# eanswer/TactileSimulation

Hardware: AMD Instinct MI355X
Metric: env-steps/sec (fwd+bwd) TactilePush batch=4096 (higher is better)
Workload: dtype f32

## Files before the change

include/tsim.h:

```cpp
#ifndef TSIM_H
#define TSIM_H
#include <stdint.h>
#ifdef __cplusplus
extern "C" {
#endif

typedef struct tsim_batch tsim_batch;
enum { TSIM_F32 = 0, TSIM_F64 = 1 };

int tsim_batch_create(const int32_t* I, const double* F, int B, int tape_capacity, int dtype, int device,
                      tsim_batch** out);
void tsim_batch_destroy(tsim_batch* b);

int tsim_ndof_r(const tsim_batch* b);
int tsim_ndof_u(const tsim_batch* b);
int tsim_ndof_var(const tsim_batch* b);
int tsim_ndof_tactile(const tsim_batch* b);
int tsim_batch_size(const tsim_batch* b);
int tsim_dtype(const tsim_batch* b);
double tsim_timestep(const tsim_batch* b);
int tsim_tape_len(const tsim_batch* b);

int tsim_update_model(tsim_batch* b, const int32_t* I, const double* F, void* stream);

// ... 57 lines not shown
                    void* g_out, void* H_out, long long* cycles, void* stream);

int tsim_debug_signature(tsim_batch* b, int t_first, int n, uint32_t* out, void* stream);

int tsim_debug_stamps(tsim_batch* b, long long* cycles);

int tsim_launch_info(const tsim_batch* b, int32_t* out);
enum { TSIM_KT_FORWARD = 0, TSIM_KT_TAXELS = 1, TSIM_KT_BACKWARD = 2, TSIM_KT_COUNT = 3 };
int tsim_kernel_timing(tsim_batch* b, int enable);
int tsim_kernel_times(tsim_batch* b, double* ms_sum, int32_t* launches);
int tsim_set_lanes_per_env(tsim_batch* b, int lanes);
int tsim_static_model(const tsim_batch* b);
int tsim_set_static(tsim_batch* b, int allow);
const char* tsim_kernel_variant(const tsim_batch* b);
enum { TSIM_OPT_PAIR_CULL = 1, TSIM_OPT_VALUE_TRIALS = 2, TSIM_OPT_TRIAL_HELPERS = 3, TSIM_OPT_VALUE_FIRST = 4, TSIM_OPT_CROSS_KINKS = 5, TSIM_OPT_EVAL_BUDGET = 6,
       TSIM_OPT_ALL_DEFAULT = 7, TSIM_OPT_FRAME_RECORDS = 8 };
int tsim_set_option(tsim_batch* b, int option, int value);
int tsim_get_option(const tsim_batch* b, int option);

int tsim_last_evals(tsim_batch* b, int32_t* host_out);
int tsim_last_helper_trials(tsim_batch* b, int32_t* host_out);

#define TSIM_KINK_FACTOR 1000.0
#define TSIM_KINK_LS 4
#define TSIM_KINK_MAX 6
int tsim_set_solver_options(tsim_batch* b, int cross_kinks, int eval_budget);
int tsim_last_gnorm(tsim_batch* b, float* host_out);

const char* tsim_last_error(void);

#ifdef __cplusplus
// ... 4 lines not shown
```

tactilesimulation_amd/csrc/tsim_batch.h:

```cpp
#pragma once
#include <hip/hip_runtime.h>
#include <cstdint>
#include <string>
#include <vector>
#include "../../include/tsim.h"
#include "tsim_launch.h"

static thread_local std::string g_err;
static int fail(const std::string& m) { g_err = m; return 1; }
#define HIPCHK(x) do { hipError_t e_ = (x); if (e_ != hipSuccess) return fail(std::string(#x) + ": " + hipGetErrorString(e_)); } while (0)

struct DeviceGuard {
  int prev = -1; bool ok = true;
  explicit DeviceGuard(int dev) {
    if (hipGetDevice(&prev) != hipSuccess) prev = -1;
    if (prev != dev) ok = hipSetDevice(dev) == hipSuccess; else prev = -1;
  }
  ~DeviceGuard() { if (prev >= 0) (void)hipSetDevice(prev); }
};
#define TS_DEVICE(b) DeviceGuard guard_((b)->device); if (!guard_.ok) return fail("hipSetDevice(" + std::to_string((b)->device) + ") failed")

static bool capturing(hipStream_t st) {
  hipStreamCaptureStatus cs = hipStreamCaptureStatusNone;
  return hipStreamIsCapturing(st, &cs) != hipSuccess || cs != hipStreamCaptureStatusNone;
// ... 28 lines not shown
  DevBuf evals;
  DevBuf helped;
  DevBuf gnorm;
  int cross_kinks = 0, eval_budget = 0;
  DevBuf order; int order_valid = 0;
  DevBuf order_ep; int order_ep_n = 0;
  DevBuf prev; int has_prev = 0;
  DevBuf poseR, poseD; int nspt;
  int has_exp;
  int t_cur, record;
  int lpe_forced;
  int nsched;
  int stage_cpt;
  int n_simd;
  int last_frame_rec = 0;
  int value_trials = 2;
  int trial_helpers = 1;
  int value_first = 1;
  bool ab_no_episode_lpt = false, ab_inkernel_readout = false, ab_no_free_run = false, ab_lockstep = false, ab_taxels_per_record = false, ab_no_envtab_cpt = false, ab_no_default_opts = false, ab_inkernel_frame_out = false; int ab_bwd_lpe = 0, ab_lpt_deal = 2;
  int pair_cull = 1;
  int static_id = 0, static_exact = 0, env_struct_ok = 0, no_static = 0;
  DevBuf dKmask, dFlag;
  DevBuf fposeR, fposeD; int fpose_frames = 0;
  int pose_valid = 0;
  int pose_off = 0;
  int tt_off = 0;
  int tax_slots = 0;
  size_t esz;
  std::vector<CacheEntry> cache;
  std::vector<void*> pool;
  std::vector<void*> retired;
  long long* bwd_stamps = nullptr;
  void* dLdp = nullptr; DevBuf zbuf, pgpart; int pg_chunks = 0;
  int pg_groups = TS_PG_CONTACT; DevBuf pgbpart;
  DevBuf tan_src; size_t tan_src_reals = 0; int tan_src_captured = 0;
  DevBuf pg_slots;
  int adj_kernel = -1, adj_passes = 0;
  int kt_on = 0;
  std::vector<KtPair> kt;
  std::vector<hipEvent_t> kt_free;
};
template <class F> static auto by_real(const tsim_batch* b, F&& f) { return by_dtype(b->dtype, f); }

struct KtScope {
  tsim_batch* b; hipStream_t st; KtPair p; bool on = false;
  KtScope(tsim_batch* b_, int kind, hipStream_t st_) : b(b_), st(st_) {
    if (!b->kt_on || b->kt.size() >= (size_t)1 << 16) return;
    if (capturing(st)) return;
    hipEvent_t e[2];
    for (int i = 0; i < 2; ++i) {
      if (!b->kt_free.empty()) { e[i] = b->kt_free.back(); b->kt_free.pop_back(); }
      else if (hipEventCreate(&e[i]) != hipSuccess) { (void)hipGetLastError(); if (i) b->kt_free.push_back(e[0]); return; }
    }
    p.a = e[0]; p.b = e[1]; p.kind = kind;
    on = hipEventRecord(p.a, st) == hipSuccess;
    if (!on) { b->kt_free.push_back(e[0]); b->kt_free.push_back(e[1]); }
  }
// ... 24 lines not shown
```

tactilesimulation_amd/csrc/tsim_hip.hip:

```cpp
#include <hip/hip_runtime.h>
#include <cstdio>
#include <cstdlib>
#include <cstring>
#include <cmath>
#include <algorithm>
#include <string>
#include <vector>
#include "../../include/tsim.h"
#include "tsim_eval.h"
#include "tsim_policy_push.h"
#include "tsim_static_pusher.h"


#include "tsim_kernels.h"
#include "tsim_param_grad.h"
#include "tsim_launch.h"
#include "tsim_batch.h"

__global__ void __launch_bounds__(1024) k_order_by_evals(const int* evals, int* order, int B, int ns, int lo, int span, int deal) {
  __shared__ int hist[64], base[64];
  const int t = threadIdx.x;
  if (t < 64) hist[t] = 0;
  __syncthreads();
  auto bin = [lo, span](int ev) { return min(max((ev - lo) * 64 / span, 0), 63); };
// ... 159 lines not shown
  for (int t = (int)blockIdx.y * a.slice + (int)threadIdx.x; t < te; t += 256 * TS_TAX_UNROLL) {
    V3<R> xa[TS_TAX_UNROLL];
#pragma unroll
    for (int r = 0; r < TS_TAX_UNROLL; ++r) {
      const int tr = min(t + 256 * r, te - 1);
      xa[r] = mk3<R>(tax[tr], tax[tr + ntax], tax[tr + 2 * ntax]);
    }
#pragma unroll
    for (int r = 0; r < TS_TAX_UNROLL; ++r)
      if (t + 256 * r < te) taxel(t + 256 * r, xa[r]);
  }
}

enum { TXS_RPB = 16, TXS_MAXK = 8, TXS_MAXS = 4, TXS_MAX_TAXELS = 1024 };
template <class R>
__global__ void __launch_bounds__(256) k_taxels_small(TaxArgs<R> a, int nrec) {
  const int rec0 = blockIdx.x * TXS_RPB, nr_ = min((int)TXS_RPB, nrec - rec0);
  const int ntax = a.ntax, nsensor = a.nsensor, nspt = a.nspt;
  __shared__ int sEnd[TXS_MAXS], sKb[TXS_MAXS], sNsp[TXS_MAXS], sPrim[TXS_MAXK], sPair[TXS_MAXK], sSlot[TXS_RPB];
  __shared__ R sSf[TXS_RPB][TXS_MAXS * TSIM_SF_SIZE], sShape[TXS_RPB][TXS_MAXK * 4], sP[TXS_RPB][TXS_MAXK * TP_R_SIZE];
  __shared__ double sD[TXS_RPB][TXS_MAXK * TP_D_SIZE];
  __shared__ __attribute__((aligned(16))) R sC[TXS_RPB][TXS_MAXK * 4];
  __shared__ R sX[3 * TXS_MAX_TAXELS];
  const R* tax = a.F + a.foff_taxel;
  for (int i = threadIdx.x; i < 3 * ntax; i += 256) sX[i] = tax[i];
  const int* TT = a.I + a.tt_off;
  for (int i = threadIdx.x; i < nsensor; i += 256) { sEnd[i] = TT[3 * i]; sKb[i] = TT[3 * i + 1]; sNsp[i] = TT[3 * i + 2]; }
  for (int i = threadIdx.x; i < nspt; i += 256) { sPrim[i] = TT[3 * nsensor + 2 * i]; sPair[i] = TT[3 * nsensor + 2 * i + 1]; }
  for (int i = threadIdx.x; i < nr_; i += 256) { const int fr = (rec0 + i) / a.B; sSlot[i] = a.tac_slot ? a.tac_slot[fr] : fr; }
  for (int i = threadIdx.x; i < nr_ * nspt * TP_R_SIZE; i += 256) { const int r = i / (nspt * TP_R_SIZE), e = i % (nspt * TP_R_SIZE); sP[r][e] = a.poseR[(size_t)(rec0 + r) * nspt * TP_R_SIZE + e]; }
  for (int i = threadIdx.x; i < nr_ * nspt * TP_D_SIZE; i += 256) { const int r = i / (nspt * TP_D_SIZE), e = i % (nspt * TP_D_SIZE); sD[r][e] = a.poseD[(size_t)(rec0 + r) * nspt * TP_D_SIZE + e]; }
  for (int i = threadIdx.x; i < nr_ * nsensor * TSIM_SF_SIZE; i += 256) {
    const int r = i / (nsensor * TSIM_SF_SIZE), e = i % (nsensor * TSIM_SF_SIZE);
    const R* F = a.Fenv ? a.Fenv + (size_t)((rec0 + r) % a.B) * a.fstride : a.F;
    sSf[r][e] = F[a.foff_sensor + e];
  }
  __syncthreads();
  for (int i = threadIdx.x; i < nr_ * nspt * 4; i += 256) {
    const int r = i / (nspt * 4), e = i % (nspt * 4);
    const R* F = a.Fenv ? a.Fenv + (size_t)((rec0 + r) % a.B) * a.fstride : a.F;
    sShape[r][e] = F[a.foff_pair + sPair[e >> 2] * TSIM_PF_SIZE + TSIM_PF_SHAPE + (e & 3)];
  }
  __syncthreads();
  for (int i = threadIdx.x; i < nr_ * nspt; i += 256) { const int r = i / nspt, k = i % nspt; taxel_bound<R>(sP[r] + k * TP_R_SIZE, sPrim[k], sShape[r] + k * 4, sC[r] + 4 * k); }
  __syncthreads();
  for (int item = threadIdx.x; item < nr_ * ntax; item += 256) {
    const int r = item / ntax, t = item - r * ntax;
    const int tslot = sSlot[r];
    if (tslot < 0) continue;
    R* out = a.tac_out + ((size_t)tslot * a.B + (rec0 + r) % a.B) * 3 * ntax;
    taxel_eval<R>(t, mk3<R>(sX[t], sX[t + ntax], sX[t + 2 * ntax]), nsensor, sEnd, sKb, sNsp, sPrim, sSf[r], sShape[r], sP[r], sD[r], sC[r], tax, ntax, out);
  }
}

template <class R> struct SigArgs { const int* I; const R* F; const R* Fenv; int fstride; int B, t_first, n; const R* tape; unsigned* out; int stage_cpt; int tk; };

__device__ __forceinline__ unsigned wave_sum_u32(unsigned x) {
  for (int off = 32; off > 0; off >>= 1) x += (unsigned)lane_gather((int)x, (int)threadIdx.x ^ off);
  return x;
}

template <class R>
__global__ void __launch_bounds__(TS_WAVE) k_signature(SigArgs<R> a) {
  extern __shared__ __attribute__((aligned(16))) unsigned char smem_raw[];
  R* lds = reinterpret_cast<R*>(smem_raw);
// ... 337 lines not shown
}
template <class R> static BwdArgs<R> bwd_args(const tsim_batch* b) {
  BwdArgs<R> a{};
  a.I = b->dI; a.F = (const R*)b->dF; a.Fenv = (const R*)b->dFenv; a.fstride = b->nfrec; a.B = b->B; a.t_end = b->t_cur;
  a.tape = (const R*)b->tape; a.lamq = (R*)b->lamq; a.lamv = (R*)b->lamv; a.stage_cpt = b->stage_cpt; a.cull = b->pair_cull; a.tk = b->tape_k;
  return a;
}

enum { TS_POSE_EMIT_MIN_TAXELS = 4096 };
static bool pose_emit(tsim_batch* b, hipStream_t st) {
  pose_invalidate(b, st);
  return !b->pose_off && b->nspt > 0 && b->poseR && b->ntax >= TS_POSE_EMIT_MIN_TAXELS;
}

static bool taxels_supported(const tsim_batch* b) { return b->ntax > 0 && b->nspt > 0 && b->nspt <= TX_MAXK && b->I[TSIM_IH_NSENSOR] <= TX_MAXS; }
template <class R>
static int launch_taxels(tsim_batch* b, const void* poseR, const double* poseD, int frames, const int32_t* tac_slot, void* tac_out, hipStream_t st) {
  if (b->tax_slots == 0) {
    int per_cu = 0;
    const hipError_t e_ = hipOccupancyMaxActiveBlocksPerMultiprocessor(&per_cu, k_taxels<R>, 256, 0);
    b->tax_slots = (e_ == hipSuccess && per_cu > 0 ? per_cu : 4) * (b->n_simd / 4);
  }
  const long long nrec = (long long)frames * b->B;
  if (nrec >= 4 * TXS_RPB && b->ntax <= TXS_MAX_TAXELS && b->nspt <= TXS_MAXK && b->I[TSIM_IH_NSENSOR] <= TXS_MAXS && !b->ab_taxels_per_record) {
    TaxArgs<R> t{b->dI, (const R*)b->dF, (const R*)b->dFenv, b->nfrec, (const R*)poseR, poseD, b->nspt, (R*)tac_out, 0, b->B, tac_slot,
                 b->ntax, b->I[TSIM_IH_NSENSOR], b->I[TSIM_IH_FOFF_SENSOR], b->I[TSIM_IH_FOFF_PAIR], b->I[TSIM_IH_FOFF_TAXEL], b->tt_off};
    hipLaunchKernelGGL(k_taxels_small<R>, dim3((unsigned)((nrec + TXS_RPB - 1) / TXS_RPB)), dim3(256), 0, st, t, (int)nrec);
    HIPCHK(hipGetLastError());
    return 0;
  }
  const int per_env = (int)std::max<long long>(1, std::min<long long>(b->tax_slots / nrec, (b->ntax + 255) / 256));
  const int slice = ((b->ntax + per_env - 1) / per_env + 255) / 256 * 256;
  const dim3 tgrid((unsigned)nrec, (b->ntax + slice - 1) / slice);
  TaxArgs<R> t{b->dI, (const R*)b->dF, (const R*)b->dFenv, b->nfrec, (const R*)poseR, poseD, b->nspt, (R*)tac_out, slice, b->B, tac_slot,
               b->ntax, b->I[TSIM_IH_NSENSOR], b->I[TSIM_IH_FOFF_SENSOR], b->I[TSIM_IH_FOFF_PAIR], b->I[TSIM_IH_FOFF_TAXEL], b->tt_off};
  hipLaunchKernelGGL(k_taxels<R>, tgrid, dim3(256), 0, st, t);
  HIPCHK(hipGetLastError());
  return 0;
}

template <class R>
static int launch_forward(tsim_batch* b, const void* u, int nframes, const int32_t* tac_slot, int nsub, void* q_out, void* qd_out, void* var_out, void* tac_out, int32_t* status, hipStream_t st) {
  FwdArgs<R> a = fwd_args<R>(b);
  a.nsub = nsub; a.nframes = nframes; a.tac_slot = tac_slot; a.u = (const R*)u;
  a.q_out = (R*)q_out; a.qd_out = (R*)qd_out; a.var_out = (R*)var_out; a.tac_out = (R*)tac_out; a.status = status;
// ... 14 lines not shown
      if (rc) defer = false;
    }
  }
  if (defer) { a.fposeR = (R*)b->fposeR; a.fposeD = b->fposeD; }
  a.free_run = (defer || !tac_out || b->ntax == 0) && !b->ab_no_free_run;
  a.lockstep = b->ab_lockstep ? 1 : 0;
  if (a.lockstep) a.free_run = 0;
  TsPlan plan = ts_plan(b, TS_K_FORWARD, false, 0);
  if (b->record && !plan.fused) b->tape_k_ok = 0;
  const TsPlan fr_plan = ts_plan(b, TS_K_FRAME_RECORDS, false, 0);
  const bool frame_rec = defer && a.free_run && b->record && nframes > 1 && plan.fused && !emit && !b->ab_inkernel_frame_out &&
                         fr_plan.variant == plan.variant && fr_plan.lpe == plan.lpe;
  a.frame_rec = frame_rec ? 1 : 0;
  plan.frame_rec = frame_rec;
  b->last_frame_rec = !frame_rec ? 0 : (plan.frame_rec && plan.default_opts) ? 2 : 1;
  { KtScope kt_(b, TSIM_KT_FORWARD, st); if (!ts_launch<false, R>(plan, st, a)) return fail("no k_forward instantiation for the launch plan"); }
  HIPCHK(hipGetLastError());
  if (defer) {
    KtScope kt_(b, TSIM_KT_TAXELS, st);
    if (frame_rec) {
      TsPlan p = fr_plan;
      const int nblk = (int)p.grid, chunks = std::max(1, std::min(nframes, b->n_simd / std::max(nblk, 1))), fpc = (nframes + chunks - 1) / chunks;
      p.grid = (unsigned)(nblk * ((nframes + fpc - 1) / fpc));
      if (!ts_launch<false, R>(p, st, a, fpc)) return fail("no k_frame_records instantiation for the launch plan");
      HIPCHK(hipGetLastError());
    }
    if (launch_taxels<R>(b, b->fposeR, b->fposeD, nframes, tac_slot, tac_out, st)) return 1;
  }
  b->pose_valid = emit ? 1 : 0;
  if (b->B >= 256) {
    const int ns = TS_WAVE / plan.lpe, nsv = (b->B % ns == 0) ? ns : 1;
    if (nframes > 1) {
      const int n = nframes * nsub;
      hipLaunchKernelGGL(k_order_by_evals, dim3(1), dim3(1024), 0, st, (const int*)b->evals, b->order_ep, b->B, nsv, 2 * n, std::max(1, 5 * n / 2), b->ab_lpt_deal);
      b->order_ep_n = n; b->order_valid = 0;
    } else {
      hipLaunchKernelGGL(k_order_by_evals, dim3(1), dim3(1024), 0, st, (const int*)b->evals, b->order, b->B, nsv, 0, 64, b->ab_lpt_deal);
      b->order_valid = 1;
    }
    HIPCHK(hipGetLastError());
  } else if (nframes > 1) b->order_valid = 0;
  return 0;
// ... 246 lines not shown
  b->rec = ts_rec(nr, nu, (int)b->esz, b->tape_k);
  if (lds_bytes_for(b, 1) > 64 * 1024) { delete b; return fail("model needs more than 64 KiB of LDS per environment"); }
  decide_stage_cpt(b);
  b->nspt = b->I[TSIM_IH_NSPRIM];
  size_t tape_bytes = (size_t)(tape_capacity + 1) * B * b->rec * b->esz;
  if (hipMalloc(&b->dI, (b->I.size() + b->nsched) * sizeof(int32_t)) != hipSuccess || hipMalloc(&b->dF, b->F.size() * b->esz) != hipSuccess ||
      hipMalloc(&b->tape, tape_bytes) != hipSuccess || hipMalloc(&b->lamq, (size_t)2 * B * nr * b->esz) != hipSuccess ||
      hipMalloc(&b->lamv, (size_t)2 * B * nr * b->esz) != hipSuccess || hipMalloc(&b->evals, (size_t)B * sizeof(int)) != hipSuccess || hipMalloc((void**)&b->helped, (size_t)B * sizeof(int)) != hipSuccess || hipMemset(b->helped, 0, (size_t)B * sizeof(int)) != hipSuccess || hipMalloc((void**)&b->gnorm, (size_t)B * sizeof(float)) != hipSuccess || hipMalloc(&b->order, (size_t)B * sizeof(int)) != hipSuccess || hipMalloc((void**)&b->order_ep, (size_t)B * sizeof(int)) != hipSuccess || hipMalloc(&b->prev, (size_t)B * 2 * nr * sizeof(double)) != hipSuccess ||
      (b->nspt > 0 && (hipMalloc(&b->poseR, (size_t)B * b->nspt * TP_R_SIZE * b->esz) != hipSuccess || hipMalloc((void**)&b->poseD, (size_t)B * b->nspt * TP_D_SIZE * sizeof(double)) != hipSuccess))) {
    tsim_batch_destroy(b);
    return fail("hipMalloc failed (tape bytes = " + std::to_string(tape_bytes) + ")");
  }
  if (hipMemset(b->tape, 0, tape_bytes) != hipSuccess || hipMemset(b->lamq, 0, (size_t)2 * B * nr * b->esz) != hipSuccess ||
      hipMemset(b->lamv, 0, (size_t)2 * B * nr * b->esz) != hipSuccess) { tsim_batch_destroy(b); return fail("hipMemset failed"); }
  if (upload_model(b, nullptr)) { tsim_batch_destroy(b); return 1; }
  *out = b;
  return 0;
}

void tsim_batch_destroy(tsim_batch* b) {
  if (!b) return;
  DeviceGuard guard_(b->device);
  for (auto& e : b->cache) (void)hipFree(e.buf);
  for (void* p : b->pool) (void)hipFree(p);
  for (void* p : b->retired) (void)hipFree(p);
  for (auto& k : b->kt) { (void)hipEventDestroy(k.a); (void)hipEventDestroy(k.b); }
  for (hipEvent_t e : b->kt_free) (void)hipEventDestroy(e);
  (void)hipFree(b->tape);
  delete b;
}

int tsim_ndof_r(const tsim_batch* b) { return b->nr; }
int tsim_ndof_u(const tsim_batch* b) { return b->nu; }
int tsim_ndof_var(const tsim_batch* b) { return 3 * b->nvar; }
int tsim_ndof_tactile(const tsim_batch* b) { return 3 * b->ntax; }
int tsim_batch_size(const tsim_batch* b) { return b->B; }
int tsim_dtype(const tsim_batch* b) { return b->dtype; }
double tsim_timestep(const tsim_batch* b) { return b->F[TSIM_FH_H]; }
int tsim_tape_len(const tsim_batch* b) { return b->record ? b->t_cur : 0; }
int tsim_launch_info(const tsim_batch* b, int32_t* out) { return plan_info(ts_plan(b, TS_K_FORWARD, false, 0), out); }
int tsim_tangent_launch_info(const tsim_batch* b, int ndir, int with_dtables, int32_t* out) {
  if (!b || !out) return fail("tangent_launch_info: null argument");
// ... 49 lines not shown
  if (option == TSIM_OPT_PAIR_CULL) { b->pair_cull = value != 0; return 0; }
  if (option == TSIM_OPT_VALUE_TRIALS) { if (value < 0) return fail("set_option: TSIM_OPT_VALUE_TRIALS >= 0"); b->value_trials = value; return 0; }
  if (option == TSIM_OPT_TRIAL_HELPERS) { b->trial_helpers = value != 0; return 0; }
  if (option == TSIM_OPT_VALUE_FIRST) { b->value_first = value != 0; return 0; }
  return fail("set_option: unknown option " + std::to_string(option));
}
int tsim_get_option(const tsim_batch* b, int option) {
  if (option == TSIM_OPT_PAIR_CULL) return b->pair_cull;
  if (option == TSIM_OPT_VALUE_TRIALS) return b->value_trials;
  if (option == TSIM_OPT_TRIAL_HELPERS) return b->trial_helpers;
  if (option == TSIM_OPT_VALUE_FIRST) return b->value_first;
  if (option == TSIM_OPT_CROSS_KINKS) return b->cross_kinks;
  if (option == TSIM_OPT_EVAL_BUDGET) return b->eval_budget;
  if (option == TSIM_OPT_ALL_DEFAULT) return default_options(b) ? 1 : 0;
  if (option == TSIM_OPT_FRAME_RECORDS) return b->last_frame_rec;
  return -1;
}
int tsim_set_solver_options(tsim_batch* b, int cross_kinks, int eval_budget) {
  if (eval_budget < 0) return fail("set_solver_options: negative evaluation budget");
  b->cross_kinks = cross_kinks != 0;
  b->eval_budget = eval_budget;
  return 0;
}
int tsim_last_gnorm(tsim_batch* b, float* host_out) {
  TS_DEVICE(b);
  if (hipMemcpy(host_out, b->gnorm, (size_t)b->B * sizeof(float), hipMemcpyDeviceToHost) != hipSuccess) return fail("last_gnorm: copy failed");
  return 0;
}
int tsim_last_helper_trials(tsim_batch* b, int32_t* host_out) {
  TS_DEVICE(b);
// ... 364 lines not shown
```

tactilesimulation_amd/csrc/tsim_kernels.h:

```cpp
#pragma once
#include <hip/hip_runtime.h>
#include "../../include/tsim.h"
#include "tsim_eval.h"
#include "tsim_policy_push.h"

template <class MS, class C> __device__ __forceinline__ int ts_integrator(const C& c) {
  if constexpr (std::is_void<MS>::value) return ts_u(c.I[TSIM_IH_INTEGRATOR]); else return MS::Iv(TSIM_IH_INTEGRATOR);
}
template <class MS> constexpr int ts_static_nr() { if constexpr (std::is_void<MS>::value) return 0; else return MS::Iv(TSIM_IH_NR); }

__host__ __device__ inline int ts_qw(int esz) { return 8 / esz; }
__host__ __device__ inline int ts_rec(int nr, int nu, int esz, int tk) { return (ts_qw(esz) * nr + nr + nr * nr + nu + (tk ? nr * nr : 0) + 1) & ~1; }
template <class R> __device__ __forceinline__ double* rec_q(R* rec) { return reinterpret_cast<double*>(rec); }
template <class R> __device__ __forceinline__ const double* rec_q(const R* rec) { return reinterpret_cast<const double*>(rec); }
template <class R> __device__ __forceinline__ int rec_qd(int nr) { return ts_qw((int)sizeof(R)) * nr; }
template <class R> __device__ __forceinline__ int rec_H(int nr) { return ts_qw((int)sizeof(R)) * nr + nr; }
template <class R> __device__ __forceinline__ int rec_u(int nr) { return ts_qw((int)sizeof(R)) * nr + nr + nr * nr; }
template <class R> __device__ __forceinline__ int rec_K(int nr, int nu) { return ts_qw((int)sizeof(R)) * nr + nr + nr * nr + nu; }

template <int LPE, class R>
__device__ __forceinline__ void readout(const Ctx<R>& c, int lane, int env, bool wr_var, bool wr, bool has_var, bool has_tac, R* var_out, R* tac_out, int tb = 0, int te = 0x7fffffff) {
  if (has_var && wr_var) {
    for (int e = lane; e < c.nvar; e += LPE) {
      const int l = c.I[c.off_var + e * TSIM_VI_SIZE + TSIM_VI_LINK];
// ... 35 lines not shown
        R o0 = R(0), o1 = R(0), o2 = R(0);
        if (Fl.x != R(0) || Fl.y != R(0) || Fl.z != R(0)) {
          o0 = Fl.x * tp[3 * c.ntax] + Fl.y * tp[4 * c.ntax] + Fl.z * tp[5 * c.ntax];
          o1 = Fl.x * tp[6 * c.ntax] + Fl.y * tp[7 * c.ntax] + Fl.z * tp[8 * c.ntax];
          o2 = Fl.x * tp[9 * c.ntax] + Fl.y * tp[10 * c.ntax] + Fl.z * tp[11 * c.ntax];
        }
        if (j0 == 0) { o[0] = o0; o[1] = o1; o[2] = o2; } else { o[0] += o0; o[1] += o1; o[2] += o2; }
      }
    }
  }
}

__device__ __forceinline__ float ts_trial_point(float base, float alpha, float dq) { return __builtin_fmaf(alpha, dq, base); }
__device__ __forceinline__ double ts_trial_point(double base, double alpha, double dq) { return __builtin_fma(alpha, dq, base); }
enum { TP_R_SIZE = 18, TP_D_SIZE = 12 };
template <class R> struct FwdArgs {
  const int* I; const R* F; const R* Fenv; int fstride;
  int B, nsub, record, t0;
  int tk = 0;
  int nframes;
  const int* tac_slot;
  R* tape; const R* u;
  R *q_out, *qd_out, *var_out, *tac_out; int* status; int* evals;
  const int* order;
  double* prev; int has_prev;
  int stage_cpt;
  int cross_kinks;
  int eval_budget;
  float* gnorm;
  PushPolicy<R> pol;
// ... 362 lines not shown
#ifdef TS_ROUND_STATS
    if (lane == 0) { if (a.gnorm) a.gnorm[env] = (float)(clock64() - rs_t0_); if (a.status) a.status[env] = rounds_; }
    if (lane == 0 && a.helped) a.helped[env] = (int)(fe_cycles_ < (1ll << 23) - 1 ? fe_cycles_ : (1ll << 23) - 1) * 256 + (fe_execs_ < 255 ? fe_execs_ : 255);
#endif
  }
}
#undef helpers_on
#undef TS_OPT
#undef TS_RECORD
template <class R, int NRM, bool EXPJ, int LPE, bool POLICY = false, class MS = void>
__global__ void TS_KLB k_forward(FwdArgs<R> a) { ts_forward<R, NRM, EXPJ, LPE, POLICY, MS>(a); }
template <class R, int NRM, int LPE, class MS>
__global__ void TS_KLB k_forward_fr(FwdArgs<R> a) { ts_forward<R, NRM, false, LPE, false, TsFrameRecords<TsDefaultOpts<MS>>>(a); }

template <class R, int LPE, class MS>
__global__ void TS_KLB k_frame_records(FwdArgs<R> a, int fpc) {
  extern __shared__ __attribute__((aligned(16))) unsigned char smem_raw[];
  R* lds = reinterpret_cast<R*>(smem_raw);
  constexpr int NS = TS_WAVE / LPE;
  const int slot = threadIdx.x / LPE, lane = threadIdx.x % LPE;
  const int nblk = (a.B + NS - 1) / NS, chunk = blockIdx.x / nblk;
  const int eidx = (blockIdx.x - chunk * nblk) * NS + slot;
  const bool valid = eidx < a.B;
  const int env = min(eidx, a.B - 1);
  Ctx<R> c; ctx_init<R, MS>(c, a.I, a.F, lds, NS, slot, lane, LPE, false, a.Fenv ? a.Fenv + (size_t)env * a.fstride : nullptr);
  const int nr = c.nr, REC = ts_rec(nr, c.nu, (int)sizeof(R), a.tk);
  init_world(c, lane, LPE);
  const int f0 = chunk * fpc, f1 = min(f0 + fpc, a.nframes);
  double qn = 0.0; R qdn = R(0);
  const R* st = a.tape + ((size_t)(a.t0 + (f0 + 1) * a.nsub) * a.B + env) * REC;
  const size_t frame_stride = (size_t)a.nsub * a.B * REC;
  if (f0 < f1 && lane < nr) { qn = rec_q(st)[lane]; qdn = st[rec_qd<R>(nr) + lane]; }
  for (int f = f0; f < f1; ++f) {
    const int tslot = a.tac_slot ? a.tac_slot[f] : f;
    TS_SYNC();
    if (lane < nr) { c.qD[lane] = qn; c.q0D[lane] = qn; c.q[lane] = (R)qn; c.qd[lane] = qdn; c.qd0[lane] = qdn; c.qa[lane] = R(0); }
    st += frame_stride;
    if (f + 1 < f1 && lane < nr) { qn = rec_q(st)[lane]; qdn = st[rec_qd<R>(nr) + lane]; }
    TS_SYNC();
// ... 279 lines not shown
```

tactilesimulation_amd/csrc/tsim_launch.h:

```cpp
#pragma once
#include <type_traits>
#include "tsim_kernels.h"
#include "tsim_param_grad.h"
#include "tsim_tangent.h"
#include "tsim_tangent_closed.h"
#include "tsim_frame_jacobian.h"
#include "tsim_tactile_jacobian.h"
#include "tsim_param_jacobian.h"
#include "tsim_static_pusher.h"

enum TsKernel { TS_K_FORWARD, TS_K_BACKWARD, TS_K_BACKWARD_Z, TS_K_DEBUG_EVAL, TS_K_PARAM_GRAD, TS_K_PARAM_GRAD_BODY, TS_K_FRAME_RECORDS,
                TS_K_CLOSED_BACKWARD_Z,
                TS_K_TANGENT,
                TS_K_TANGENT_BODY,
                TS_K_CLOSED_TANGENT,
                TS_K_FRAME_JACOBIAN,
                TS_K_TACTILE_JACOBIAN,
                TS_K_PARAM_JACOBIAN };
enum { TS_KM_GENERIC = 0, TS_KM_STATIC = 1, TS_KM_PARAM = 2 };
using TsParamPusher = TsParam<TsStaticPusher>;

struct TsPlan {
  int kernel = TS_K_FORWARD, variant = TS_KM_GENERIC;
  int nrm = 8; bool expj = false; int lpe = TS_WAVE;
// ... 32 lines not shown
template <int N> using TsInt = std::integral_constant<int, N>;
template <bool B> using TsBool = std::integral_constant<bool, B>;

template <class MS, bool POLICY, class R> struct TsLaunch {
  template <int K, class F> static bool shape(const TsPlan& p, F&& f) {
    if (p.kernel != K || p.policy != POLICY) return false;
    auto at = [&](auto nrm, auto expj, auto lpe) {
      if constexpr (ts_instantiated(K, ts_view_nrm<MS>(), sizeof(R) == 4, POLICY, false, nrm, expj, lpe)) { f(nrm, expj, lpe); return true; }
      else return false;
    };
    auto lanes = [&](auto nrm, auto expj) { return p.lpe == 16 ? at(nrm, expj, TsInt<16>()) : p.lpe == 32 ? at(nrm, expj, TsInt<32>()) : p.lpe == 64 && at(nrm, expj, TsInt<64>()); };
    if (p.expj) return p.nrm == 16 && lanes(TsInt<16>(), TsBool<true>());
    return p.nrm == 8 ? lanes(TsInt<8>(), TsBool<false>()) : p.nrm == 16 && lanes(TsInt<16>(), TsBool<false>());
  }
  static bool run(const TsPlan& p, hipStream_t st, const FwdArgs<R>& a);
  static bool run(const TsPlan& p, hipStream_t st, const FwdArgs<R>& a, int fpc);
  static bool run(const TsPlan& p, hipStream_t st, const BwdArgs<R>& a, R* zsave = nullptr);
  static bool run_closed_z(const TsPlan& p, hipStream_t st, const BwdArgs<R>& a, R* zsave);
  static bool run(const TsPlan& p, hipStream_t st, const DbgArgs<R>& a);
  static bool run(const TsPlan& p, hipStream_t st, const PgArgs<R>& a);
  static bool run(const TsPlan& p, hipStream_t st, const PgBodyArgs<R>& a);
  static bool run(const TsPlan& p, hipStream_t st, const TanArgs<R>& a);
  static bool run(const TsPlan& p, hipStream_t st, const TanBodyArgs<R>& a);
  static bool run(const TsPlan& p, hipStream_t st, const FjArgs<R>& a);
  static bool run(const TsPlan& p, hipStream_t st, const TjArgs<R>& a);
  static bool run(const TsPlan& p, hipStream_t st, const PjArgs<R>& a);
  static bool run_tangent_src(const TsPlan& p, hipStream_t st, const TanArgs<R>& a);
  static bool run_closed_tangent(const TsPlan& p, hipStream_t st, const TanClosedArgs<R>& a);
};

template <class MS, bool POLICY, class R> bool TsLaunch<MS, POLICY, R>::run(const TsPlan& p, hipStream_t st, const FwdArgs<R>& a) {
  return shape<TS_K_FORWARD>(p, [&](auto nrm, auto expj, auto lpe) {
    if constexpr (ts_instantiated(TS_K_FORWARD, ts_view_nrm<MS>(), sizeof(R) == 4, POLICY, true, nrm, expj, lpe)) {
      if (p.default_opts && p.frame_rec) {
        if constexpr (!POLICY && ts_static_fused<MS, R>()) { hipLaunchKernelGGL((k_forward_fr<R, nrm, lpe, MS>), dim3(p.grid), dim3(TS_WAVE), p.lds, st, a); return; }
      }
      if (p.default_opts) { hipLaunchKernelGGL((k_forward<R, nrm, expj, lpe, POLICY, TsDefaultOpts<MS>>), dim3(p.grid), dim3(TS_WAVE), p.lds, st, a); return; }
    }
    hipLaunchKernelGGL((k_forward<R, nrm, expj, lpe, POLICY, MS>), dim3(p.grid), dim3(TS_WAVE), p.lds, st, a);
  });
}
template <class MS, bool POLICY, class R> bool TsLaunch<MS, POLICY, R>::run(const TsPlan& p, hipStream_t st, const FwdArgs<R>& a, int fpc) {
  if constexpr (!POLICY && ts_static_fused<MS, R>())
    return shape<TS_K_FRAME_RECORDS>(p, [&](auto, auto, auto lpe) { hipLaunchKernelGGL((k_frame_records<R, lpe, MS>), dim3(p.grid), dim3(TS_WAVE), p.lds, st, a, fpc); });
  else return false;
}
template <class MS, bool POLICY, class R> bool TsLaunch<MS, POLICY, R>::run(const TsPlan& p, hipStream_t st, const BwdArgs<R>& a, R* zsave) {
  if (p.kernel == TS_K_CLOSED_BACKWARD_Z) return run_closed_z(p, st, a, zsave);
  if (p.kernel == TS_K_BACKWARD_Z)
    return shape<TS_K_BACKWARD_Z>(p, [&](auto nrm, auto expj, auto lpe) { hipLaunchKernelGGL((k_backward_z<R, nrm, expj, lpe, POLICY, MS>), dim3(p.grid), dim3(TS_WAVE), p.lds, st, a, zsave); });
  return shape<TS_K_BACKWARD>(p, [&](auto nrm, auto expj, auto lpe) { hipLaunchKernelGGL((k_backward<R, nrm, expj, lpe, POLICY, MS>), dim3(p.grid), dim3(TS_WAVE), p.lds, st, a); });
}
template <class MS, bool POLICY, class R> bool TsLaunch<MS, POLICY, R>::run_closed_z(const TsPlan& p, hipStream_t st, const BwdArgs<R>& a, R* zsave) {
  return shape<TS_K_CLOSED_BACKWARD_Z>(p, [&](auto nrm, auto expj, auto lpe) { hipLaunchKernelGGL((k_closed_backward_z<R, nrm, expj, lpe, MS>), dim3(p.grid), dim3(TS_WAVE), p.lds, st, a, zsave); });
}
template <class MS, bool POLICY, class R> bool TsLaunch<MS, POLICY, R>::run(const TsPlan& p, hipStream_t st, const DbgArgs<R>& a) {
  return shape<TS_K_DEBUG_EVAL>(p, [&](auto, auto, auto lpe) { hipLaunchKernelGGL((k_debug_eval<R, lpe, MS>), dim3(p.grid), dim3(TS_WAVE), p.lds, st, a); });
}
template <class MS, bool POLICY, class R> bool TsLaunch<MS, POLICY, R>::run(const TsPlan& p, hipStream_t st, const PgArgs<R>& a) {
// ... 65 lines not shown
```

tactilesimulation_amd/host/batch.py:

```python
import ctypes as C

import numpy as np
import torch

from . import capi
from ..model.compiler import CompiledModel, load_model


def _ptr(t):
    return C.c_void_p(t.data_ptr()) if t is not None else None


class BatchSim:
    def __init__(self, model, batch_size, device="cuda:0", dtype=torch.float32, tape_capacity=512):
        if isinstance(model, str):
            model = load_model(model)
        assert isinstance(model, CompiledModel)
        self.model = model
        self.device = torch.device(device)
        if self.device.type != "cuda":
            raise RuntimeError("BatchSim needs a GPU device (got %s); the HIP path has no CPU fallback" % device)
        if dtype not in (torch.float32, torch.float64):
            raise ValueError("dtype must be float32 or float64")
        self.dtype = dtype
# ... 320 lines not shown
        capi.check(capi.lib().tsim_set_solver_options(self._h, int(bool(cross_kinks)), int(eval_budget)))

    def set_lanes_per_env(self, lanes):
        capi.check(capi.lib().tsim_set_lanes_per_env(self._h, int(lanes)))

    def static_model(self):
        return capi.lib().tsim_static_model(self._h)

    def set_static(self, allow):
        capi.check(capi.lib().tsim_set_static(self._h, int(bool(allow))))

    def kernel_variant(self):
        return capi.lib().tsim_kernel_variant(self._h).decode()

    OPT_PAIR_CULL, OPT_VALUE_TRIALS, OPT_TRIAL_HELPERS, OPT_VALUE_FIRST, OPT_CROSS_KINKS, OPT_EVAL_BUDGET, OPT_ALL_DEFAULT, OPT_FRAME_RECORDS = 1, 2, 3, 4, 5, 6, 7, 8

    def set_option(self, option, value):
        capi.check(capi.lib().tsim_set_option(self._h, int(option), int(value)))

    def get_option(self, option):
        return capi.lib().tsim_get_option(self._h, int(option))

    KERNEL_KINDS = ("k_forward", "k_taxels", "k_backward")

    def kernel_timing(self, enable=True):
        capi.check(capi.lib().tsim_kernel_timing(self._h, int(bool(enable))))

    def kernel_times(self):
        ms, n = (C.c_double * 3)(), (C.c_int32 * 3)()
        capi.check(capi.lib().tsim_kernel_times(self._h, ms, n))
# ... 27 lines not shown
```

tactilesimulation_amd/host/buildhash.py:

```python
import hashlib
import os


def digest(paths, flags=()):
    h = hashlib.sha256()
    for f in flags:
        h.update(f.encode() + b"\0")
    for p in paths:
        h.update(os.path.basename(p).encode() + b"\0")
        with open(p, "rb") as fh:
            h.update(fh.read())
    return h.hexdigest()


def sidecar(lib):
    return lib + ".buildhash"


def read(lib):
    try:
        return open(sidecar(lib)).read().strip()
    except OSError:
        return None

# ... 88 lines not shown
            json.dump(table, fh, indent=0, sort_keys=True)
        return table
    finally:
        shutil.rmtree(tmp, ignore_errors=True)


def kernel_name(kernel, dtype, nr, has_exp, lanes, variant, policy=False, default_opts=False):
    nrm, expj, lpe = (16, True, 64) if has_exp else ((8 if nr <= 8 else 16), False, lanes)
    if variant != "generic":
        nrm = 8
    ms = {"generic": ("v", "void"), "static:pusher": ("14TsStaticPusher", "TsStaticPusher"), "param:pusher": ("7TsParamI14TsStaticPusherE", "TsParam<TsStaticPusher>")}[variant]
    if default_opts and kernel == "k_forward" and variant != "generic" and dtype == "f32" and lpe == 16:
        ms = ("13TsDefaultOptsI%sE" % ms[0], "TsDefaultOpts<%s>" % ms[1])
    r = {"f32": ("f", "float"), "f64": ("d", "double")}[dtype]
    if kernel == "k_frame_records":
        return ("_Z15k_frame_recordsI%sLi%dE%sEv7FwdArgsIT_Ei" % (r[0], lpe, ms[0]), "k_frame_records<%s, LPE=%d, %s>" % (r[1], lpe, ms[1]))
    if kernel == "k_forward_fr":
        return ("_Z12k_forward_frI%sLi%dELi%dE%sEv7FwdArgsIT_E" % (r[0], nrm, lpe, ms[0]), "k_forward_fr<%s, NRM=%d, LPE=%d, %s>" % (r[1], nrm, lpe, ms[1]))
    if kernel == "k_closed_backward_z":
        back = {"generic": 1, "static:pusher": 2, "param:pusher": 4}[variant]
        return ("_Z19k_closed_backward_zI%sLi%dELb%dELi%dE%sEv7BwdArgsIT_EPS%d_" % (r[0], nrm, int(expj), lpe, ms[0], back),
                "k_closed_backward_z<%s, NRM=%d, EXPJ=%s, LPE=%d, %s>" % (r[1], nrm, str(expj).lower(), lpe, ms[1]))
    args = {"k_forward": "7FwdArgs", "k_backward": "7BwdArgs"}[kernel]
    mangled = "_Z%d%sI%sLi%dELb%dELi%dELb%dE%sEv%sIT_E" % (len(kernel), kernel, r[0], nrm, int(expj), lpe, int(policy), ms[0], args)
    return mangled, "%s<%s, NRM=%d, EXPJ=%s, LPE=%d, POLICY=%s, %s>" % (kernel, r[1], nrm, str(expj).lower(), lpe, str(policy).lower(), ms[1])
```

Baseline: 33.54 million.

## Split forward into heavy and light env ranges overlapped on two streams

The forward launch is split into two parts by env order. A small heavy subset of blocks runs on the main stream while the remaining light envs run on a second stream, each followed by its own frame-record and taxel readout. Both k_frame_records and k_taxels_small gain a sub-range argument so they can process a permuted slice of environments. The aim is to overlap the tail of the forward kernel with readout work instead of serialising them, at the cost of extra stream and event overhead and more complex indexing.

```diff
diff --git a/include/tsim.h b/include/tsim.h
--- a/include/tsim.h
+++ b/include/tsim.h
@@ -95,7 +95,7 @@
 int tsim_set_static(tsim_batch* b, int allow);
 const char* tsim_kernel_variant(const tsim_batch* b);
 enum { TSIM_OPT_PAIR_CULL = 1, TSIM_OPT_VALUE_TRIALS = 2, TSIM_OPT_TRIAL_HELPERS = 3, TSIM_OPT_VALUE_FIRST = 4, TSIM_OPT_CROSS_KINKS = 5, TSIM_OPT_EVAL_BUDGET = 6,
-       TSIM_OPT_ALL_DEFAULT = 7, TSIM_OPT_FRAME_RECORDS = 8 };
+       TSIM_OPT_ALL_DEFAULT = 7, TSIM_OPT_FRAME_RECORDS = 8, TSIM_OPT_FORWARD_SPLIT = 9 };
 int tsim_set_option(tsim_batch* b, int option, int value);
 int tsim_get_option(const tsim_batch* b, int option);
 
diff --git a/tactilesimulation_amd/csrc/tsim_batch.h b/tactilesimulation_amd/csrc/tsim_batch.h
--- a/tactilesimulation_amd/csrc/tsim_batch.h
+++ b/tactilesimulation_amd/csrc/tsim_batch.h
@@ -66,6 +66,10 @@
   int stage_cpt;
   int n_simd;
   int last_frame_rec = 0;
+  hipStream_t split_st = nullptr;
+  hipEvent_t split_fork = nullptr;
+  hipEvent_t split_join = nullptr;
+  int last_fwd_split = 0;
   int value_trials = 2;
   int trial_helpers = 1;
   int value_first = 1;
@@ -93,6 +97,12 @@
   std::vector<hipEvent_t> kt_free;
 };
 template <class F> static auto by_real(const tsim_batch* b, F&& f) { return by_dtype(b->dtype, f); }
+static void split_release(tsim_batch* b) {
+  if (b->split_st) (void)hipStreamDestroy(b->split_st);
+  if (b->split_fork) (void)hipEventDestroy(b->split_fork);
+  if (b->split_join) (void)hipEventDestroy(b->split_join);
+  b->split_st = nullptr; b->split_fork = b->split_join = nullptr;
+}
 
 struct KtScope {
   tsim_batch* b; hipStream_t st; KtPair p; bool on = false;
diff --git a/tactilesimulation_amd/csrc/tsim_hip.hip b/tactilesimulation_amd/csrc/tsim_hip.hip
--- a/tactilesimulation_amd/csrc/tsim_hip.hip
+++ b/tactilesimulation_amd/csrc/tsim_hip.hip
@@ -197,10 +197,10 @@
 
 enum { TXS_RPB = 16, TXS_MAXK = 8, TXS_MAXS = 4, TXS_MAX_TAXELS = 1024 };
 template <class R>
-__global__ void __launch_bounds__(256) k_taxels_small(TaxArgs<R> a, int nrec) {
+__global__ void __launch_bounds__(256) k_taxels_small(TaxArgs<R> a, int nrec, TsSubRange sub) {
   const int rec0 = blockIdx.x * TXS_RPB, nr_ = min((int)TXS_RPB, nrec - rec0);
   const int ntax = a.ntax, nsensor = a.nsensor, nspt = a.nspt;
-  __shared__ int sEnd[TXS_MAXS], sKb[TXS_MAXS], sNsp[TXS_MAXS], sPrim[TXS_MAXK], sPair[TXS_MAXK], sSlot[TXS_RPB];
+  __shared__ int sEnd[TXS_MAXS], sKb[TXS_MAXS], sNsp[TXS_MAXS], sPrim[TXS_MAXK], sPair[TXS_MAXK], sSlot[TXS_RPB], sEnv[TXS_RPB], sRec[TXS_RPB];
   __shared__ R sSf[TXS_RPB][TXS_MAXS * TSIM_SF_SIZE], sShape[TXS_RPB][TXS_MAXK * 4], sP[TXS_RPB][TXS_MAXK * TP_R_SIZE];
   __shared__ double sD[TXS_RPB][TXS_MAXK * TP_D_SIZE];
   __shared__ __attribute__((aligned(16))) R sC[TXS_RPB][TXS_MAXK * 4];
@@ -210,18 +210,22 @@
   const int* TT = a.I + a.tt_off;
   for (int i = threadIdx.x; i < nsensor; i += 256) { sEnd[i] = TT[3 * i]; sKb[i] = TT[3 * i + 1]; sNsp[i] = TT[3 * i + 2]; }
   for (int i = threadIdx.x; i < nspt; i += 256) { sPrim[i] = TT[3 * nsensor + 2 * i]; sPair[i] = TT[3 * nsensor + 2 * i + 1]; }
-  for (int i = threadIdx.x; i < nr_; i += 256) { const int fr = (rec0 + i) / a.B; sSlot[i] = a.tac_slot ? a.tac_slot[fr] : fr; }
-  for (int i = threadIdx.x; i < nr_ * nspt * TP_R_SIZE; i += 256) { const int r = i / (nspt * TP_R_SIZE), e = i % (nspt * TP_R_SIZE); sP[r][e] = a.poseR[(size_t)(rec0 + r) * nspt * TP_R_SIZE + e]; }
-  for (int i = threadIdx.x; i < nr_ * nspt * TP_D_SIZE; i += 256) { const int r = i / (nspt * TP_D_SIZE), e = i % (nspt * TP_D_SIZE); sD[r][e] = a.poseD[(size_t)(rec0 + r) * nspt * TP_D_SIZE + e]; }
+  for (int i = threadIdx.x; i < nr_; i += 256) {
+    const int fr = (rec0 + i) / sub.n, ei = sub.e0 + (rec0 + i) - fr * sub.n, env = sub.order ? sub.order[ei] : ei;
+    sSlot[i] = a.tac_slot ? a.tac_slot[fr] : fr; sEnv[i] = env; sRec[i] = fr * a.B + env;
+  }
+  __syncthreads();
+  for (int i = threadIdx.x; i < nr_ * nspt * TP_R_SIZE; i += 256) { const int r = i / (nspt * TP_R_SIZE), e = i % (nspt * TP_R_SIZE); sP[r][e] = a.poseR[(size_t)sRec[r] * nspt * TP_R_SIZE + e]; }
+  for (int i = threadIdx.x; i < nr_ * nspt * TP_D_SIZE; i += 256) { const int r = i / (nspt * TP_D_SIZE), e = i % (nspt * TP_D_SIZE); sD[r][e] = a.poseD[(size_t)sRec[r] * nspt * TP_D_SIZE + e]; }
   for (int i = threadIdx.x; i < nr_ * nsensor * TSIM_SF_SIZE; i += 256) {
     const int r = i / (nsensor * TSIM_SF_SIZE), e = i % (nsensor * TSIM_SF_SIZE);
-    const R* F = a.Fenv ? a.Fenv + (size_t)((rec0 + r) % a.B) * a.fstride : a.F;
+    const R* F = a.Fenv ? a.Fenv + (size_t)sEnv[r] * a.fstride : a.F;
     sSf[r][e] = F[a.foff_sensor + e];
   }
   __syncthreads();
   for (int i = threadIdx.x; i < nr_ * nspt * 4; i += 256) {
     const int r = i / (nspt * 4), e = i % (nspt * 4);
-    const R* F = a.Fenv ? a.Fenv + (size_t)((rec0 + r) % a.B) * a.fstride : a.F;
+    const R* F = a.Fenv ? a.Fenv + (size_t)sEnv[r] * a.fstride : a.F;
     sShape[r][e] = F[a.foff_pair + sPair[e >> 2] * TSIM_PF_SIZE + TSIM_PF_SHAPE + (e & 3)];
   }
   __syncthreads();
@@ -231,7 +235,7 @@
     const int r = item / ntax, t = item - r * ntax;
     const int tslot = sSlot[r];
     if (tslot < 0) continue;
-    R* out = a.tac_out + ((size_t)tslot * a.B + (rec0 + r) % a.B) * 3 * ntax;
+    R* out = a.tac_out + ((size_t)tslot * a.B + sEnv[r]) * 3 * ntax;
     taxel_eval<R>(t, mk3<R>(sX[t], sX[t + ntax], sX[t + 2 * ntax]), nsensor, sEnd, sKb, sNsp, sPrim, sSf[r], sShape[r], sP[r], sD[r], sC[r], tax, ntax, out);
   }
 }
@@ -599,21 +603,26 @@
 }
 
 static bool taxels_supported(const tsim_batch* b) { return b->ntax > 0 && b->nspt > 0 && b->nspt <= TX_MAXK && b->I[TSIM_IH_NSENSOR] <= TX_MAXS; }
-template <class R>
-static int launch_taxels(tsim_batch* b, const void* poseR, const double* poseD, int frames, const int32_t* tac_slot, void* tac_out, hipStream_t st) {
+static bool taxels_small(const tsim_batch* b, long long nrec) {
+  return nrec >= 4 * TXS_RPB && b->ntax <= TXS_MAX_TAXELS && b->nspt <= TXS_MAXK && b->I[TSIM_IH_NSENSOR] <= TXS_MAXS && !b->ab_taxels_per_record;
+}
+template <class R>
+static int launch_taxels(tsim_batch* b, const void* poseR, const double* poseD, int frames, const int32_t* tac_slot, void* tac_out, hipStream_t st, const TsSubRange* sub = nullptr) {
   if (b->tax_slots == 0) {
     int per_cu = 0;
     const hipError_t e_ = hipOccupancyMaxActiveBlocksPerMultiprocessor(&per_cu, k_taxels<R>, 256, 0);
     b->tax_slots = (e_ == hipSuccess && per_cu > 0 ? per_cu : 4) * (b->n_simd / 4);
   }
-  const long long nrec = (long long)frames * b->B;
-  if (nrec >= 4 * TXS_RPB && b->ntax <= TXS_MAX_TAXELS && b->nspt <= TXS_MAXK && b->I[TSIM_IH_NSENSOR] <= TXS_MAXS && !b->ab_taxels_per_record) {
+  const TsSubRange all{nullptr, 0, b->B};
+  const long long nrec = (long long)frames * (sub ? sub->n : b->B);
+  if (taxels_small(b, nrec)) {
     TaxArgs<R> t{b->dI, (const R*)b->dF, (const R*)b->dFenv, b->nfrec, (const R*)poseR, poseD, b->nspt, (R*)tac_out, 0, b->B, tac_slot,
                  b->ntax, b->I[TSIM_IH_NSENSOR], b->I[TSIM_IH_FOFF_SENSOR], b->I[TSIM_IH_FOFF_PAIR], b->I[TSIM_IH_FOFF_TAXEL], b->tt_off};
-    hipLaunchKernelGGL(k_taxels_small<R>, dim3((unsigned)((nrec + TXS_RPB - 1) / TXS_RPB)), dim3(256), 0, st, t, (int)nrec);
+    hipLaunchKernelGGL(k_taxels_small<R>, dim3((unsigned)((nrec + TXS_RPB - 1) / TXS_RPB)), dim3(256), 0, st, t, (int)nrec, sub ? *sub : all);
     HIPCHK(hipGetLastError());
     return 0;
   }
+  if (sub) return fail("launch_taxels: a sub-range of the environments is k_taxels_small's");
   const int per_env = (int)std::max<long long>(1, std::min<long long>(b->tax_slots / nrec, (b->ntax + 255) / 256));
   const int slice = ((b->ntax + per_env - 1) / per_env + 255) / 256 * 256;
   const dim3 tgrid((unsigned)nrec, (b->ntax + slice - 1) / slice);
@@ -658,18 +667,63 @@
   a.frame_rec = frame_rec ? 1 : 0;
   plan.frame_rec = frame_rec;
   b->last_frame_rec = !frame_rec ? 0 : (plan.frame_rec && plan.default_opts) ? 2 : 1;
-  { KtScope kt_(b, TSIM_KT_FORWARD, st); if (!ts_launch<false, R>(plan, st, a)) return fail("no k_forward instantiation for the launch plan"); }
-  HIPCHK(hipGetLastError());
-  if (defer) {
-    KtScope kt_(b, TSIM_KT_TAXELS, st);
-    if (frame_rec) {
-      TsPlan p = fr_plan;
-      const int nblk = (int)p.grid, chunks = std::max(1, std::min(nframes, b->n_simd / std::max(nblk, 1))), fpc = (nframes + chunks - 1) / chunks;
-      p.grid = (unsigned)(nblk * ((nframes + fpc - 1) / fpc));
-      if (!ts_launch<false, R>(p, st, a, fpc)) return fail("no k_frame_records instantiation for the launch plan");
+  const int ns_ = TS_WAVE / plan.lpe;
+  auto frame_records = [&](hipStream_t s, const TsSubRange& sub) {
+    TsPlan p = fr_plan;
+    const int nblk = (sub.n + ns_ - 1) / ns_, chunks = std::max(1, std::min(nframes, b->n_simd / std::max(nblk, 1))), fpc = (nframes + chunks - 1) / chunks;
+    p.grid = (unsigned)(nblk * ((nframes + fpc - 1) / fpc));
+    return ts_launch<false, R>(p, s, a, fpc, sub);
+  };
+  const int nblk_f = (int)plan.grid, wh = std::max(1, nblk_f / 8);
+  const bool split = frame_rec && b->split_st && a.order && a.order == (const int*)b->order_ep && b->B % ns_ == 0 && nblk_f <= b->n_simd && nblk_f >= 64 &&
+                     taxels_small(b, (long long)nframes * wh * ns_) && !capturing(st);
+  b->last_fwd_split = split ? 1 : 0;
+  if (split) {
+    const TsSubRange heavy{a.order, 0, wh * ns_}, light{a.order, wh * ns_, b->B - wh * ns_};
+    auto forward = [&](hipStream_t s, unsigned grid, const FwdArgs<R>& fa) -> int {
+      TsPlan p = plan; p.grid = grid;
+      if (!ts_launch<false, R>(p, s, fa)) return fail("no k_forward instantiation for the launch plan");
       HIPCHK(hipGetLastError());
-    }
-    if (launch_taxels<R>(b, b->fposeR, b->fposeD, nframes, tac_slot, tac_out, st)) return 1;
+      return 0;
+    };
+    auto read_out = [&](hipStream_t s, const TsSubRange& sub) -> int {
+      if (!frame_records(s, sub)) return fail("no k_frame_records instantiation for the launch plan");
+      HIPCHK(hipGetLastError());
+      return launch_taxels<R>(b, b->fposeR, b->fposeD, nframes, tac_slot, tac_out, s, &sub);
+    };
+    int rc;
+    {
+      KtScope kt_(b, TSIM_KT_FORWARD, st);
+      HIPCHK(hipEventRecord(b->split_fork, st));
+      HIPCHK(hipStreamWaitEvent(b->split_st, b->split_fork, 0));
+      rc = forward(st, (unsigned)wh, a);
+    }
+    if (!rc) {
+      FwdArgs<R> al = a; al.order = a.order + light.e0;
+      rc = forward(b->split_st, (unsigned)(nblk_f - wh), al);
+    }
+    if (!rc) rc = read_out(b->split_st, light);
+    const hipError_t e_rec = hipEventRecord(b->split_join, b->split_st);
+    hipError_t e_wait;
+    {
+      KtScope kt_(b, TSIM_KT_TAXELS, st);
+      if (!rc) rc = read_out(st, heavy);
+      e_wait = e_rec == hipSuccess ? hipStreamWaitEvent(st, b->split_join, 0) : hipStreamSynchronize(b->split_st);
+    }
+    if (rc) return rc;
+    HIPCHK(e_rec);
+    HIPCHK(e_wait);
+  } else {
+    { KtScope kt_(b, TSIM_KT_FORWARD, st); if (!ts_launch<false, R>(plan, st, a)) return fail("no k_forward instantiation for the launch plan"); }
+    HIPCHK(hipGetLastError());
+    if (defer) {
+      KtScope kt_(b, TSIM_KT_TAXELS, st);
+      if (frame_rec) {
+        if (!frame_records(st, TsSubRange{nullptr, 0, b->B})) return fail("no k_frame_records instantiation for the launch plan");
+        HIPCHK(hipGetLastError());
+      }
+      if (launch_taxels<R>(b, b->fposeR, b->fposeD, nframes, tac_slot, tac_out, st)) return 1;
+    }
   }
   b->pose_valid = emit ? 1 : 0;
   if (b->B >= 256) {
@@ -946,6 +1000,13 @@
   if (hipMemset(b->tape, 0, tape_bytes) != hipSuccess || hipMemset(b->lamq, 0, (size_t)2 * B * nr * b->esz) != hipSuccess ||
       hipMemset(b->lamv, 0, (size_t)2 * B * nr * b->esz) != hipSuccess) { tsim_batch_destroy(b); return fail("hipMemset failed"); }
   if (upload_model(b, nullptr)) { tsim_batch_destroy(b); return 1; }
+  if (B >= 64 && !getenv("TSIM_NO_FORWARD_SPLIT")) {
+    if (hipStreamCreateWithFlags(&b->split_st, hipStreamNonBlocking) != hipSuccess || hipEventCreateWithFlags(&b->split_fork, hipEventDisableTiming) != hipSuccess ||
+        hipEventCreateWithFlags(&b->split_join, hipEventDisableTiming) != hipSuccess) {
+      (void)hipGetLastError();
+      split_release(b);
+    }
+  }
   *out = b;
   return 0;
 }
@@ -958,6 +1019,7 @@
   for (void* p : b->retired) (void)hipFree(p);
   for (auto& k : b->kt) { (void)hipEventDestroy(k.a); (void)hipEventDestroy(k.b); }
   for (hipEvent_t e : b->kt_free) (void)hipEventDestroy(e);
+  split_release(b);
   (void)hipFree(b->tape);
   delete b;
 }
@@ -1037,6 +1099,7 @@
   if (option == TSIM_OPT_EVAL_BUDGET) return b->eval_budget;
   if (option == TSIM_OPT_ALL_DEFAULT) return default_options(b) ? 1 : 0;
   if (option == TSIM_OPT_FRAME_RECORDS) return b->last_frame_rec;
+  if (option == TSIM_OPT_FORWARD_SPLIT) return b->last_fwd_split;
   return -1;
 }
 int tsim_set_solver_options(tsim_batch* b, int cross_kinks, int eval_budget) {
diff --git a/tactilesimulation_amd/csrc/tsim_kernels.h b/tactilesimulation_amd/csrc/tsim_kernels.h
--- a/tactilesimulation_amd/csrc/tsim_kernels.h
+++ b/tactilesimulation_amd/csrc/tsim_kernels.h
@@ -73,6 +73,7 @@
 __device__ __forceinline__ float ts_trial_point(float base, float alpha, float dq) { return __builtin_fmaf(alpha, dq, base); }
 __device__ __forceinline__ double ts_trial_point(double base, double alpha, double dq) { return __builtin_fma(alpha, dq, base); }
 enum { TP_R_SIZE = 18, TP_D_SIZE = 12 };
+struct TsSubRange { const int* order; int e0, n; };
 template <class R> struct FwdArgs {
   const int* I; const R* F; const R* Fenv; int fstride;
   int B, nsub, record, t0;
@@ -465,15 +466,16 @@
 __global__ void TS_KLB k_forward_fr(FwdArgs<R> a) { ts_forward<R, NRM, false, LPE, false, TsFrameRecords<TsDefaultOpts<MS>>>(a); }
 
 template <class R, int LPE, class MS>
-__global__ void TS_KLB k_frame_records(FwdArgs<R> a, int fpc) {
+__global__ void TS_KLB k_frame_records(FwdArgs<R> a, int fpc, TsSubRange sub) {
   extern __shared__ __attribute__((aligned(16))) unsigned char smem_raw[];
   R* lds = reinterpret_cast<R*>(smem_raw);
   constexpr int NS = TS_WAVE / LPE;
   const int slot = threadIdx.x / LPE, lane = threadIdx.x % LPE;
-  const int nblk = (a.B + NS - 1) / NS, chunk = blockIdx.x / nblk;
+  const int nblk = (sub.n + NS - 1) / NS, chunk = blockIdx.x / nblk;
   const int eidx = (blockIdx.x - chunk * nblk) * NS + slot;
-  const bool valid = eidx < a.B;
-  const int env = min(eidx, a.B - 1);
+  const bool valid = eidx < sub.n;
+  const int ei = sub.e0 + min(eidx, sub.n - 1);
+  const int env = sub.order ? sub.order[ei] : ei;
   Ctx<R> c; ctx_init<R, MS>(c, a.I, a.F, lds, NS, slot, lane, LPE, false, a.Fenv ? a.Fenv + (size_t)env * a.fstride : nullptr);
   const int nr = c.nr, REC = ts_rec(nr, c.nu, (int)sizeof(R), a.tk);
   init_world(c, lane, LPE);
diff --git a/tactilesimulation_amd/csrc/tsim_launch.h b/tactilesimulation_amd/csrc/tsim_launch.h
--- a/tactilesimulation_amd/csrc/tsim_launch.h
+++ b/tactilesimulation_amd/csrc/tsim_launch.h
@@ -70,7 +70,7 @@
     return p.nrm == 8 ? lanes(TsInt<8>(), TsBool<false>()) : p.nrm == 16 && lanes(TsInt<16>(), TsBool<false>());
   }
   static bool run(const TsPlan& p, hipStream_t st, const FwdArgs<R>& a);
-  static bool run(const TsPlan& p, hipStream_t st, const FwdArgs<R>& a, int fpc);
+  static bool run(const TsPlan& p, hipStream_t st, const FwdArgs<R>& a, int fpc, TsSubRange sub);
   static bool run(const TsPlan& p, hipStream_t st, const BwdArgs<R>& a, R* zsave = nullptr);
   static bool run_closed_z(const TsPlan& p, hipStream_t st, const BwdArgs<R>& a, R* zsave);
   static bool run(const TsPlan& p, hipStream_t st, const DbgArgs<R>& a);
@@ -96,9 +96,9 @@
     hipLaunchKernelGGL((k_forward<R, nrm, expj, lpe, POLICY, MS>), dim3(p.grid), dim3(TS_WAVE), p.lds, st, a);
   });
 }
-template <class MS, bool POLICY, class R> bool TsLaunch<MS, POLICY, R>::run(const TsPlan& p, hipStream_t st, const FwdArgs<R>& a, int fpc) {
+template <class MS, bool POLICY, class R> bool TsLaunch<MS, POLICY, R>::run(const TsPlan& p, hipStream_t st, const FwdArgs<R>& a, int fpc, TsSubRange sub) {
   if constexpr (!POLICY && ts_static_fused<MS, R>())
-    return shape<TS_K_FRAME_RECORDS>(p, [&](auto, auto, auto lpe) { hipLaunchKernelGGL((k_frame_records<R, lpe, MS>), dim3(p.grid), dim3(TS_WAVE), p.lds, st, a, fpc); });
+    return shape<TS_K_FRAME_RECORDS>(p, [&](auto, auto, auto lpe) { hipLaunchKernelGGL((k_frame_records<R, lpe, MS>), dim3(p.grid), dim3(TS_WAVE), p.lds, st, a, fpc, sub); });
   else return false;
 }
 template <class MS, bool POLICY, class R> bool TsLaunch<MS, POLICY, R>::run(const TsPlan& p, hipStream_t st, const BwdArgs<R>& a, R* zsave) {
diff --git a/tactilesimulation_amd/host/batch.py b/tactilesimulation_amd/host/batch.py
--- a/tactilesimulation_amd/host/batch.py
+++ b/tactilesimulation_amd/host/batch.py
@@ -358,6 +358,7 @@
         return capi.lib().tsim_kernel_variant(self._h).decode()
 
     OPT_PAIR_CULL, OPT_VALUE_TRIALS, OPT_TRIAL_HELPERS, OPT_VALUE_FIRST, OPT_CROSS_KINKS, OPT_EVAL_BUDGET, OPT_ALL_DEFAULT, OPT_FRAME_RECORDS = 1, 2, 3, 4, 5, 6, 7, 8
+    OPT_FORWARD_SPLIT = 9
 
     def set_option(self, option, value):
         capi.check(capi.lib().tsim_set_option(self._h, int(option), int(value)))
diff --git a/tactilesimulation_amd/host/buildhash.py b/tactilesimulation_amd/host/buildhash.py
--- a/tactilesimulation_amd/host/buildhash.py
+++ b/tactilesimulation_amd/host/buildhash.py
@@ -126,7 +126,7 @@
         ms = ("13TsDefaultOptsI%sE" % ms[0], "TsDefaultOpts<%s>" % ms[1])
     r = {"f32": ("f", "float"), "f64": ("d", "double")}[dtype]
     if kernel == "k_frame_records":
-        return ("_Z15k_frame_recordsI%sLi%dE%sEv7FwdArgsIT_Ei" % (r[0], lpe, ms[0]), "k_frame_records<%s, LPE=%d, %s>" % (r[1], lpe, ms[1]))
+        return ("_Z15k_frame_recordsI%sLi%dE%sEv7FwdArgsIT_Ei10TsSubRange" % (r[0], lpe, ms[0]), "k_frame_records<%s, LPE=%d, %s>" % (r[1], lpe, ms[1]))
     if kernel == "k_forward_fr":
         return ("_Z12k_forward_frI%sLi%dELi%dE%sEv7FwdArgsIT_E" % (r[0], nrm, lpe, ms[0]), "k_forward_fr<%s, NRM=%d, LPE=%d, %s>" % (r[1], nrm, lpe, ms[1]))
     if kernel == "k_closed_backward_z":
```

Result: faster. 34.62 million (median of 6 runs) (+3.2%).
